# QuantumSavory/LDPCDecoders.jl

Hardware: AMD Instinct MI355X
Metric: decoded syndromes/sec (batchdecode!, 50 iters) + achieved HBM GB/s fraction (higher is better)
Workload: dtype f64

## Files before the change

### include/ldpc_mi355x_debug.h

```cpp
#ifndef LDPC_MI355X_DEBUG_H
#define LDPC_MI355X_DEBUG_H

#include "ldpc_mi355x.h"

#ifdef __cplusplus
extern "C" {
#endif

ldpc_status ldpc_debug_team_plan(int64_t nnz, int64_t max_iters, int64_t batch, int32_t cache_mib, int32_t rows_dv,
                                 int32_t out[6]);

ldpc_status ldpc_debug_team_rows(int64_t s, int64_t n, const int64_t *colptr, const int64_t *rowval, int32_t members,
                                 int32_t regs_per_wave, int32_t static_quarters, int32_t *degrees, int32_t *shape,
                                 int32_t *vtab, int32_t *ctab, int32_t *lds_edge, int32_t *reg_edge);

ldpc_status ldpc_debug_team_irr(int64_t s, int64_t n, const int64_t *colptr, const int64_t *rowval, int32_t members,
                                int32_t dc_bucket, int32_t dv_bucket, int32_t *shape, int32_t *ctab2, int32_t *ptab, int32_t *ploc,
                                int32_t *lds_edge, int32_t *posmap);

ldpc_status ldpc_debug_tile_plan(int64_t s, int64_t n, int64_t rec_words, int32_t relay, int32_t kernel_variant, int32_t *tier,
                                 int32_t *tile_syndromes, int64_t *state_bytes);

ldpc_status ldpc_debug_priors_tile_plan(int64_t s, int64_t n, int64_t rec_words, int32_t schedule, int32_t kernel_variant,
                                        int32_t *tier, int32_t *tile_syndromes, int64_t *state_bytes);

ldpc_status ldpc_debug_pauli_tile_plan(int64_t s, int64_t n, int64_t rec_words, int32_t kernel_variant, int32_t *tier,
                                       int32_t *tile_syndromes, int64_t *state_bytes);

#include "ldpc_mi355x_decim_debug.h"

#include "ldpc_mi355x_pauli_relay_debug.h"

ldpc_status ldpc_debug_layer_plan(int64_t s, int64_t n, const int64_t *colptr, const int64_t *rowval, int32_t *layer_of,
                                  int32_t *K);

ldpc_status ldpc_debug_bpots_plan(int64_t s, int64_t n, int64_t nnz, int32_t max_cdeg, int32_t max_bdeg, int32_t force_node,
                                  int32_t *kernel, int32_t *logS, int64_t *lds_bytes, int32_t *budget_kib, int32_t *dc, int32_t *dv);

ldpc_status ldpc_debug_bpots_last_launch(const ldpc_bpots_decoder *dec, int32_t *path, int64_t *groups, int32_t *grid,
                                         int32_t *chunk, int32_t *per_cu);

void *ldpc_debug_process_state(void);
ldpc_status ldpc_debug_adopt_process_state(void *state);

ldpc_status ldpc_debug_div_check(int64_t count, const double *num, const double *den, double *out_core, double *out_ieee);

ldpc_status ldpc_debug_llr_check(int64_t count, const double *odds, double *out_fast, double *out_lib);

#ifdef __cplusplus
}
#endif
#endif
```

### ldpcdecoders.jl_amd/_capi.py

```python
from __future__ import annotations

import ctypes
import os
import subprocess

_HERE = os.path.dirname(os.path.abspath(__file__))
CSRC = os.path.join(_HERE, "csrc")
LIB_PATH = os.environ.get("LDPC_MI355X_LIB") or os.path.join(CSRC, "libldpc_mi355x.so")
EXP_LIB_PATH = os.environ.get("LDPC_MI355X_EXP_LIB") or os.path.join(CSRC, "libldpc_mi355x_exp.so")

LDPC_OK = 0
STATUS_NAMES = {
    0: "LDPC_OK",
    1: "LDPC_ERR_INVALID_ARGUMENT",
    2: "LDPC_ERR_NO_DEVICE",
    3: "LDPC_ERR_HIP",
    4: "LDPC_ERR_OUT_OF_MEMORY",
    5: "LDPC_ERR_UNSUPPORTED",
}

MULTI_MAX_DEVICES = 16
EXCHANGE_AUTO, EXCHANGE_COPY, EXCHANGE_RCCL, EXCHANGE_NONE = 0, 1, 2, 3


# ... 201 lines not shown
    "ldpc_debug_process_state": (vp, []),
    "ldpc_debug_adopt_process_state": (i32, [vp]),
    "ldpc_debug_team_irr": (i32, [i64, i64, vp, vp, i32, i32, i32, P(i32 * 2), vp, vp, vp, vp, vp]),
    "ldpc_debug_llr_check": (i32, [i64, vp, vp, vp]),
    "ldpc_debug_tile_plan": (i32, [i64, i64, i64, i32, i32, P(i32), P(i32), P(i64)]),
    "ldpc_debug_layer_plan": (i32, [i64, i64, vp, vp, vp, P(i32)]),
    "ldpc_debug_priors_tile_plan": (i32, [i64, i64, i64, i32, i32, P(i32), P(i32), P(i64)]),
    "ldpc_debug_pauli_tile_plan": (i32, [i64, i64, i64, i32, P(i32), P(i32), P(i64)]),
    "ldpc_debug_bpots_plan": (i32, [i64, i64, i64, i32, i32, i32, P(i32), P(i32), P(i64), P(i32), P(i32), P(i32)]),
    "ldpc_debug_bpots_last_launch": (i32, [vp, P(i32), P(i64), P(i32), P(i32), P(i32)]),
}
DECIM_API = {
    "ldpc_decim_create": (i32, [i64, i64, i64, vp, vp, vp, i64, i64, P(DecimOptions), P(vp)]),
    "ldpc_decim_destroy": (i32, [vp]),
    "ldpc_decim_kernel": (i32, [vp]),
    "ldpc_decim_tile_syndromes": (i32, [vp]),
    "ldpc_decim_last_grid": (i32, [vp]),
    "ldpc_decim_decode_batch": (i32, [vp, i64, vp, vp, vp, vp, vp, vp]),
    "ldpc_decim_decode_batch_device": (i32, [vp, i64, vp, vp, vp, vp, vp, vp, vp]),
}
DECIM_DEBUG_API = {
    "ldpc_debug_decim_tile_plan": (i32, [i64, i64, i64, i32, P(i32), P(i32), P(i64)]),
}
OSD_SEARCH_API = {
    "ldpc_osd_set_search": (i32, [vp, i32, i64, i64, vp]),
    "ldpc_osd_search_method": (i32, [vp]),
    "ldpc_osd_search_weight": (i64, [vp, i64]),
}
PAULI_RELAY_API = {
    "ldpc_pauli_relay_create": (i32, [i64, P(CSSPattern), P(CSSPattern), vp, vp, vp, i64, vp, vp, P(PauliRelayOptions), P(vp)]),
    "ldpc_pauli_relay_destroy": (i32, [vp]),
    "ldpc_pauli_relay_kernel": (i32, [vp]),
    "ldpc_pauli_relay_tile_syndromes": (i32, [vp]),
    "ldpc_pauli_relay_last_grid": (i32, [vp]),
    "ldpc_pauli_relay_decode_batch": (i32, [vp, i64, vp, vp, vp, vp, vp, vp, vp, vp]),
    "ldpc_pauli_relay_decode_batch_device": (i32, [vp, i64, vp, vp, vp, vp, vp, vp, vp, vp, vp]),
}
PAULI_RELAY_DEBUG_API = {
    "ldpc_debug_pauli_relay_tile_plan": (i32, [i64, i64, i64, i32, P(i32), P(i32), P(i64)]),
}
EXPORTED_SYMBOLS = tuple(API)
DEBUG_SYMBOLS = tuple(DEBUG_API)
DECIM_SYMBOLS = tuple(DECIM_API)
DECIM_DEBUG_SYMBOLS = tuple(DECIM_DEBUG_API)
OSD_SEARCH_SYMBOLS = tuple(OSD_SEARCH_API)
PAULI_RELAY_SYMBOLS = tuple(PAULI_RELAY_API)
PAULI_RELAY_DEBUG_SYMBOLS = tuple(PAULI_RELAY_DEBUG_API)


def build(force: bool = False) -> str:
    subprocess.check_call(["make", "-s", "-C", CSRC, "all"])
    return LIB_PATH


_LIBS = {}


def _one_hip_runtime() -> None:
    if os.environ.get("LDPC_MI355X_NO_TORCH_PRELOAD"):
        return
    try:
        import torch
    except Exception:
        pass


def lib(experiments: bool = False) -> ctypes.CDLL:
    if experiments in _LIBS:
        return _LIBS[experiments]
    path = EXP_LIB_PATH if experiments else LIB_PATH
    if not os.path.exists(path):
        raise LdpcError(2, f"{path} is not built; run `python -c 'import __graft_entry__ as g; g.build()'` "
                           "or `make -C ldpcdecoders.jl_amd/csrc`. There is no CPU fallback.")
    _one_hip_runtime()
    L = ctypes.CDLL(path)
    for group in (API, DEBUG_API, DECIM_API, DECIM_DEBUG_API, OSD_SEARCH_API, PAULI_RELAY_API, PAULI_RELAY_DEBUG_API):
        for name, (restype, argtypes) in group.items():
            fn = getattr(L, name)
            fn.restype, fn.argtypes = restype, argtypes
    other = _LIBS.get(not experiments)
    if other is not None and os.path.realpath(path) != os.path.realpath(EXP_LIB_PATH if not experiments else LIB_PATH):
        check(L.ldpc_debug_adopt_process_state(other.ldpc_debug_process_state()), L)
    _LIBS[experiments] = L
    return L


def knobs_in_env() -> bool:
    return any(k.startswith("LDPC_") and not k.startswith("LDPC_MI355X_") for k in os.environ)


def lib_for(experiments=None) -> ctypes.CDLL:
    return lib(knobs_in_env() if experiments is None else bool(experiments))


def check(status: int, L: ctypes.CDLL = None) -> None:
    if status != LDPC_OK:
        raise LdpcError(status, (L or lib()).ldpc_last_error().decode("utf-8", "replace"))
```

### ldpcdecoders.jl_amd/csrc/bp_team_kernels.hpp

```cpp
#pragma once
#include "bp_kernels.hpp"

#ifndef LDPC_TEAM_ROWS_WIDE
#define LDPC_TEAM_ROWS_WIDE 1
#endif
#ifndef LDPC_TEAM_TFORM
#define LDPC_TEAM_TFORM 1
#endif
#ifndef LDPC_TEAM_TEST_DIRECT
#define LDPC_TEAM_TEST_DIRECT 1
#endif
#ifndef LDPC_TEAM_SLEEP
#define LDPC_TEAM_SLEEP 16
#endif

namespace ldpc {


template <int DV>
struct TeamVRec {
    int pos[DV], lrow[DV], bit;
};
template <int DV>
__device__ __forceinline__ TeamVRec<DV> team_vrec_load(const int *__restrict__ vt)
// ... 67 lines not shown

struct TeamParams {
    TeamRows rows;
    int G;
    int xcds;
    int nteams;
    int pre;
    int pairs;
    int dynamic;
    unsigned int *ctl;
    u64 *mism;
    int mism_stride;
    unsigned int *fault;
    int always_release;
    int scatter;
    unsigned int count_max;
    int inject_fault;
    unsigned int ticket;
    unsigned int rollcall_ticks;
    u64 *errmask_alt;
    int ahead_min;
    int ahead_from;
    int llr_raw;
};
constexpr unsigned int kTeamRollcallFailed = 0x80000000u;

constexpr int kTeamCtlMember = 64;
constexpr int kTeamCtlWords = 64 + 32 * kTeamMaxMembers;

#ifndef LDPC_TEAM_BARRIER_COUNTER
#define LDPC_TEAM_BARRIER_COUNTER 0
#endif
__device__ __forceinline__ bool team_barrier(unsigned int *ctl, int G, int rank, unsigned int k, unsigned int *fault,
                                             unsigned int ticket, int *sh_ok, bool one_xcd, unsigned int *sh_deal)
{
    asm volatile("s_waitcnt vmcnt(0)" ::: "memory");
    __syncthreads();
    if (threadIdx.x == 0) {
        if (!one_xcd) {
            __builtin_amdgcn_fence(__ATOMIC_RELEASE, "agent");
            asm volatile("s_waitcnt vmcnt(0)" ::: "memory");
        }
        int ok = 1;
        const unsigned int prev = __hip_atomic_fetch_add(ctl, 1u, __ATOMIC_RELAXED, __HIP_MEMORY_SCOPE_AGENT);
        const bool on_counter = LDPC_TEAM_BARRIER_COUNTER && one_xcd;
        if (prev + 1u == k * (unsigned)G) {
            if (!on_counter)
                for (int m = 0; m < G; ++m)
// ... 461 lines not shown
    if (team >= nteams || team >= ntiles) return;
    const int gw = rank * W + w, GW = G * W;
    unsigned int *const ctr = tp.ctl + (size_t)team * kTeamCtlWords;
    unsigned int *const xccs = ctr + 32;
    unsigned int *const tile_queue = tp.ctl + (size_t)nteams * kTeamCtlWords;
    unsigned int epoch = 0;
    __shared__ int sh_one_xcd;
#if LDPC_TEAM_FAULT_BLOCKS
    if (tp.inject_fault == 2 && team == 0 && rank == G - 1) return;
#endif
    if (!team_rollcall(ctr + 36, G, tp.fault, tp.ticket, tp.rollcall_ticks, &sh_ok)) return;
    if (threadIdx.x == 0) {
        unsigned int xcc;
        asm volatile("s_getreg_b32 %0, hwreg(HW_REG_XCC_ID)" : "=s"(xcc));
        __hip_atomic_fetch_or(xccs, 1u << (xcc & 15u), __ATOMIC_RELAXED, __HIP_MEMORY_SCOPE_AGENT);
    }
    bool one_xcd = false, placed = false;
    constexpr bool resumed = RESUMED;
    const BPCold *const cd = p.cold;
    u64 tk_check = 0, tk_var = 0, tk_rest = 0;
    int horizon = p.max_iters;
    long long tot_iters = 0;

    for (int tile = team; tile < ntiles;) {
    double *const Mt = p.msg + (size_t)(resumed ? tile : team) * (size_t)p.slot_stride + lane;
    u64 *const mw = tp.mism + (size_t)tile * (size_t)tp.mism_stride;
    const u64 *syn = synmask + (size_t)tile * s;
    u64 *em = p.errmask + (size_t)tile * n;
    u64 *fin = p.finmask + (size_t)tile * n;
    const long long b0 = (long long)tile * kTile;
    const long long left = batch - b0;
    u64 deferred = 0;
    const u64 valid = left >= kTile ? ~0ull : ((1ull << left) - 1ull);
    const u64 never = nevermask[tile];
    u64 active = valid;
    const int it0 = (resumed && ((valid >> lane) & 1ull)) ? cd->it0[b0 + lane] : 0;
    int my_iters = 0, my_conv = 0, it = 0;

    const bool can_run_ahead = !resumed && tp.errmask_alt != nullptr && tp.ahead_min > 0;
    u64 *const em_even = em, *const em_odd = can_run_ahead ? tp.errmask_alt + (size_t)tile * n : em;
    bool have_check = false;
    bool quiet = true;

    auto check_sweep = [&](const bool first, const int skip = 0) {
        const int nch = (s + kTeamCheckChunk - 1) / kTeamCheckChunk;
        auto chunk = [&](int c) {
            const int i1 = min(s, (c + 1) * kTeamCheckChunk);
            if constexpr (LROWS) {
                typedef int v4i __attribute__((ext_vector_type(4)));
                typedef int v8i __attribute__((ext_vector_type(8)));
                constexpr int FULL = (1 << DC) - 1;
                auto one = [&](double *const M, const v4i ct, const double sg) {
                    if (RR > 0 && ct.z == FULL) {
                        if (first) check_update_regs<DC, true, TF>(ct.w, sg, r, rget, rput);
                        else check_update_regs<DC, false, TF>(ct.w, sg, r, rget, rput);
                    } else if (ct.x == FULL) {
                        if (first) check_update_exact<DC, true, TF>(Lr + (size_t)ct.y * kTile, sg, r);
                        else check_update_exact<DC, false, TF>(Lr + (size_t)ct.y * kTile, sg, r);
                    } else if (RR > 0 && ct.z != 0) {
                        if (first) check_update_onchip<DC, true, TF>(M, Lr + (size_t)ct.y * kTile, Ldummy, (unsigned int)ct.x, (unsigned int)ct.z, ct.w, sg, r, rget, rput);
                        else check_update_onchip<DC, false, TF>(M, Lr + (size_t)ct.y * kTile, Ldummy, (unsigned int)ct.x, (unsigned int)ct.z, ct.w, sg, r, rget, rput);
                    } else if (first) {
                        check_update_mixed<DC, true, TF>(M, Lr + (size_t)ct.y * kTile, (unsigned int)ct.x, sg, r);
                    } else if (ct.x == 0) {
                        check_update_exact<DC, false, TF>(M, sg, r);
                    } else {
                        check_update_mixed<DC, false, TF>(M, Lr + (size_t)ct.y * kTile, (unsigned int)ct.x, sg, r);
                    }
                };
                const int i = c * kTeamCheckChunk;
                if (LDPC_HOT(kTeamCheckChunk == 2 && i + 2 == i1)) {
                    const v8i ct = *(const v8i *)(col_ptr + 4 * i);
                    const u64 s0 = syn[i], s1 = syn[i + 1];
                    const double sg0 = ((s0 >> lane) & 1ull) ? -1.0 : 1.0, sg1 = ((s1 >> lane) & 1ull) ? -1.0 : 1.0;
                    double *const M0 = Mt + (size_t)i * DC * kTile, *const M1 = M0 + (size_t)DC * kTile;
                    if ((ct.s0 | ct.s2 | ct.s4 | ct.s6) == 0 && !first && tp.pairs) {
                        check_update_pair<DC, TF>(M0, M1, sg0, sg1);
                    } else {
                        one(M0, v4i{ct.s0, ct.s1, ct.s2, ct.s3}, sg0);
                        one(M1, v4i{ct.s4, ct.s5, ct.s6, ct.s7}, sg1);
                    }
                    return;
                }
                for (int ii = i; ii < i1; ++ii) {
                    const v4i ct = *(const v4i *)(col_ptr + 4 * ii);
                    one(Mt + (size_t)ii * DC * kTile, ct, ((syn[ii] >> lane) & 1ull) ? -1.0 : 1.0);
                }
                return;
            }
            if constexpr (IRR) {
                for (int i = c * kTeamCheckChunk; i < i1; ++i) {
                    const int e0 = row_ptr[2 * i], lb = row_ptr[2 * i + 1];
                    const int deg = row_ptr[2 * i + 2] - e0;
                    const double sigma = ((syn[i] >> lane) & 1ull) ? -1.0 : 1.0;
                    double *const M = lb >= 0 ? Lr + (size_t)lb * kTile : Mt + (size_t)e0 * kTile;
                    if (first) check_update<DC, true, true>(M, deg, sigma, r);
                    else check_update<DC, false, true>(M, deg, sigma, r);
// ... 2 lines not shown
            }
            if (kTeamCheckChunk == 2 && !first && tp.pairs && i1 == c * 2 + 2) {
                const int i = c * 2;
                const int e0 = row_ptr[i], e1 = row_ptr[i + 1], e2 = row_ptr[i + 2];
                if (e1 - e0 == DC && e2 - e1 == DC) {
                    const double sg0 = ((syn[i] >> lane) & 1ull) ? -1.0 : 1.0, sg1 = ((syn[i + 1] >> lane) & 1ull) ? -1.0 : 1.0;
                    check_update_pair<DC>(Mt + (size_t)e0 * kTile, Mt + (size_t)e1 * kTile, sg0, sg1);
                    return;
                }
            }
            for (int i = c * kTeamCheckChunk; i < i1; ++i) {
                const int e0 = row_ptr[i];
                const int deg = row_ptr[i + 1] - e0;
                const double sigma = ((syn[i] >> lane) & 1ull) ? -1.0 : 1.0;
                if (first) check_update<DC, true>(Mt + (size_t)e0 * kTile, deg, sigma, r);
                else check_update<DC, false>(Mt + (size_t)e0 * kTile, deg, sigma, r);
            }
        };
        const int mine = (nch - rank + G - 1) / G;
        const int stat = LROWS ? tp.rows.static_c : W;
        const int mirror = (LROWS && (tp.rows.flip & 1) && w >= W / 2) ? 2 * w + stat - W : -1;
        for (int l = w; l < mine;) {
            const int lc = (mirror >= 0 && l < stat) ? mirror - l : l;
            if (!(LROWS && lc < skip * W)) chunk(lc * G + rank);
            l = !tp.dynamic ? l + W : (l + W < stat ? l + W : stat + team_deal(&sh_deal[0], lane));
        }
    };
    auto check_pre = [&](const int pre) {
        if constexpr (LROWS) {
            typedef int v4i __attribute__((ext_vector_type(4)));
            constexpr int FULL = (1 << DC) - 1;
            for (int k = 0; k < pre; ++k) {
                const int c = (w + k * W) * G + rank;
                for (int i = c * kTeamCheckChunk; i < (c + 1) * kTeamCheckChunk; ++i) {
                    const v4i ct = *(const v4i *)(col_ptr + 4 * i);
                    const double sg = ((syn[i] >> lane) & 1ull) ? -1.0 : 1.0;
                    if (RR > 0 && ct.z == FULL) check_update_regs<DC, false, TF>(ct.w, sg, r, rget, rput);
                    else check_update_exact<DC, false, TF>(Lr + (size_t)ct.y * kTile, sg, r);
                }
            }
        }
    };
    auto var_sweep = [&](const bool first = false) {
        const int vb = (one_xcd || LROWS || IRR) ? 4 : 16;
        const int nch = (n + vb - 1) / vb;
        const bool cap_on = WANT_LLR && (tp.llr_raw == 4 || tp.llr_raw == 5) && ((active >> lane) & 1ull);
        const size_t cap_rows = ((size_t)n + 3) & ~(size_t)3;
        unsigned int *const cap32 = (unsigned int *)p.llr + (size_t)tile * cap_rows * kTile;
        double *const cap64 = p.llr + (size_t)tile * cap_rows * kTile;
        auto cap_at = [&](int pos) { return ((size_t)(pos >> 2) * kTile + lane) * 4 + (size_t)(pos & 3); };
        auto capture1 = [&](int pos, double T) {
            if (!cap_on) return;
            if (tp.llr_raw == 4) cap32[cap_at(pos)] = llr_hi32(T);
            else cap64[cap_at(pos)] = T;
        };
        auto capture2 = [&](int pos, double T0, double T1) {
            if (!cap_on) return;
            typedef unsigned int v2u __attribute__((ext_vector_type(2)));
            typedef double v2d __attribute__((ext_vector_type(2)));
            if (tp.llr_raw == 4) *(v2u *)(cap32 + cap_at(pos)) = v2u{llr_hi32(T0), llr_hi32(T1)};
            else *(v2d *)(cap64 + cap_at(pos)) = v2d{T0, T1};
        };
        auto capture4 = [&](int pos, const double (&T)[4]) {
            if (!cap_on) return;
            typedef unsigned int v4u __attribute__((ext_vector_type(4)));
            typedef double v2d __attribute__((ext_vector_type(2)));
            if (tp.llr_raw == 4) *(v4u *)(cap32 + cap_at(pos)) = v4u{llr_hi32(T[0]), llr_hi32(T[1]), llr_hi32(T[2]), llr_hi32(T[3])};
            else { *(v2d *)(cap64 + cap_at(pos)) = v2d{T[0], T[1]}; *(v2d *)(cap64 + cap_at(pos) + 2) = v2d{T[2], T[3]}; }
        };
        auto decide = [&](int pos, int j, double T, bool cap = true) {
            const u64 dec = __ballot(T >= 1.0);
            if (WANT_LLR) {
                if (tp.llr_raw >= 4) { if (cap) capture1(pos, T); }
                else if (tp.llr_raw == 0 && ((active >> lane) & 1ull)) p.llr[((size_t)tile * n + j) * kTile + lane] = llr_of(T, p.llr_exact);
            }
            if (lane == 0) em[j] = dec;
        };
        auto chunk = [&](int c) {
            const int j1 = min(n, (c + 1) * vb);
            int j = c * vb;
            if constexpr (LROWS) {
                constexpr int VT = team_vtab_words(DV);
                if constexpr (kFuseFirst) {
                    if (first) {
                        if (j + 4 == j1) {
                            const int *const vt = csc2csr + (size_t)j * VT;
                            const TeamVRec<DV> A = team_vrec_load<DV>(vt), B = team_vrec_load<DV>(vt + VT), C = team_vrec_load<DV>(vt + 2 * VT),
                                               D = team_vrec_load<DV>(vt + 3 * VT);
                            double T[4];
                            T[0] = bit_update_first<DV, DC, TF>(Mt, Lr, sh_first, syn, lane, A.pos, A.lrow, r, rput);
                            T[1] = bit_update_first<DV, DC, TF>(Mt, Lr, sh_first, syn, lane, B.pos, B.lrow, r, rput);
                            T[2] = bit_update_first<DV, DC, TF>(Mt, Lr, sh_first, syn, lane, C.pos, C.lrow, r, rput);
                            T[3] = bit_update_first<DV, DC, TF>(Mt, Lr, sh_first, syn, lane, D.pos, D.lrow, r, rput);
                            decide(j, A.bit & 0x7fffffff, T[0], false);
                            decide(j + 1, B.bit & 0x7fffffff, T[1], false);
                            decide(j + 2, C.bit & 0x7fffffff, T[2], false);
                            decide(j + 3, D.bit & 0x7fffffff, T[3], false);
                            capture4(j, T);
                            return;
                        }
                        for (; j < j1; ++j) {
                            const TeamVRec<DV> A = team_vrec_load<DV>(csc2csr + (size_t)j * VT);
                            decide(j, A.bit & 0x7fffffff, bit_update_first<DV, DC, TF>(Mt, Lr, sh_first, syn, lane, A.pos, A.lrow, r, rput));
                        }
                        return;
                    }
                }
                auto single = [&](const TeamVRec<DV> &a, const int pa) {
                    if (a.bit >= 0) { decide(pa, a.bit, bit_update_exact_v<DV, TF>(Mt, a.pos, r)); return; }
                    if constexpr (RR > 0) {
                        int lo = a.lrow[0];
// ... 7 lines not shown
                    int rest = -1;
#pragma unroll
                    for (int k = 1; k < DV; ++k) rest &= a.lrow[k] & b.lrow[k];
                    if ((a.bit | b.bit) >= 0 && tp.pairs) {
                        double T0, T1;
                        bit_update_pair_v<DV, TF>(Mt, a.pos, b.pos, r, T0, T1);
                        decide(pa, a.bit, T0, false);
                        decide(pa + 1, b.bit, T1, false);
                        capture2(pa, T0, T1);
                    } else if (rest == -1 && tp.pairs) {
                        double T0, T1;
                        bit_update_pair_first<DV, TF>(Mt, Lr, a.pos, a.lrow[0], b.pos, b.lrow[0], r, rget, rput, T0, T1);
                        decide(pa, a.bit & 0x7fffffff, T0, false);
                        decide(pa + 1, b.bit & 0x7fffffff, T1, false);
                        capture2(pa, T0, T1);
                    } else {
                        single(a, pa);
                        single(b, pa + 1);
                    }
                };
                int q = j;
                if (LDPC_HOT(q + 4 == j1)) {
                    const int *const vt = csc2csr + (size_t)q * VT;
                    const TeamVRec<DV> A = team_vrec_load<DV>(vt), B = team_vrec_load<DV>(vt + VT), C = team_vrec_load<DV>(vt + 2 * VT),
                                       D = team_vrec_load<DV>(vt + 3 * VT);
                    if (LDPC_HOT(tp.pairs & 2)) {
                        int rest = -1;
#pragma unroll
                        for (int k = 1; k < DV; ++k) rest &= A.lrow[k] & B.lrow[k] & C.lrow[k] & D.lrow[k];
                        if (LDPC_HOT(rest == -1)) {
                            int ps[4][DV];
#pragma unroll
                            for (int k = 0; k < DV; ++k) { ps[0][k] = A.pos[k]; ps[1][k] = B.pos[k]; ps[2][k] = C.pos[k]; ps[3][k] = D.pos[k]; }
                            const int lc[4] = {A.lrow[0], B.lrow[0], C.lrow[0], D.lrow[0]};
                            double T[4];
                            constexpr bool KINDS = LDPC_TEAM_CHUNK_KINDS < 0 ? DV == 3 : LDPC_TEAM_CHUNK_KINDS != 0;
                            const int lmin = min(min(lc[0], lc[1]), min(lc[2], lc[3])), lmax = max(max(lc[0], lc[1]), max(lc[2], lc[3]));
                            if (KINDS && RR > 0 && lmax <= -2) bit_update_multi_first<DV, 4, TF, 2>(Mt, Lr, ps, lc, r, rget, rput, T);
                            else if (KINDS && lmin >= 0) bit_update_multi_first<DV, 4, TF, 1>(Mt, Lr, ps, lc, r, rget, rput, T);
                            else bit_update_multi_first<DV, 4, TF, 0>(Mt, Lr, ps, lc, r, rget, rput, T);
                            decide(q, A.bit & 0x7fffffff, T[0], false);
                            decide(q + 1, B.bit & 0x7fffffff, T[1], false);
                            decide(q + 2, C.bit & 0x7fffffff, T[2], false);
                            decide(q + 3, D.bit & 0x7fffffff, T[3], false);
                            capture4(q, T);
                            return;
                        }
                    }
// ... 17 lines not shown
                    decide(j, bw & 0x7fffffff, T);
                }
                return;
            }
            for (; tp.pairs && j + 1 < j1; j += 2) {
                const int c0 = col_ptr[j], c1 = col_ptr[j + 1], c2 = col_ptr[j + 2];
                if (c1 - c0 != DV || c2 - c1 != DV) break;
                double T0, T1;
                bit_update_pair<DV>(Mt, csc2csr + c0, csc2csr + c1, r, T0, T1);
                decide(j, j, T0, false);
                decide(j + 1, j + 1, T1, false);
                capture2(j, T0, T1);
            }
            for (; j < j1; ++j) {
                const int c0 = col_ptr[j];
                const int deg = col_ptr[j + 1] - c0;
                decide(j, j, bit_update<DV>(Mt, csc2csr + c0, deg, r));
            }
        };
        const int mine = (nch - rank + G - 1) / G;
        const int stat = LROWS ? tp.rows.static_v : W;
        const int mirror = (LROWS && (tp.rows.flip & 2) && w >= W / 2) ? 2 * w + stat - W : -1;
        for (int l = w; l < mine;) {
            chunk(((mirror >= 0 && l < stat) ? mirror - l : l) * G + rank);
            l = !tp.dynamic ? l + W : (l + W < stat ? l + W : stat + team_deal(&sh_deal[1], lane));
        }
    };
    auto run_test = [&](const int it_t, const u64 *em_t) {
        u64 mism = 0;
#if LDPC_TEAM_TEST_SPREAD
        const int gt = w * G + rank;
#else
        const int gt = gw;
#endif
        for (int i = gt * 64 + lane; i < s; i += GW * 64) {
            u64 par = 0;
            const int e1 = LROWS ? (i + 1) * DC : row_ptr[RS * (i + 1)];
            for (int e = LROWS ? i * DC : row_ptr[RS * i]; e < e1; e += 8) {
                int jb[8];
#pragma unroll
                for (int q = 0; q < 8; ++q) jb[q] = (e + q < e1) ? edge_bit[e + q] : -1;
                u64 wv[8];
#pragma unroll
                for (int q = 0; q < 8; ++q) wv[q] = (jb[q] >= 0) ? em_t[jb[q]] : 0ull;
#pragma unroll
                for (int q = 0; q < 8; ++q) par ^= wv[q];
            }
            mism |= par ^ syn[i];
        }
        mism = wave_or(mism);
#if LDPC_TEAM_TEST_DIRECT
        if (lane == 0 && mism) __hip_atomic_fetch_or(&mw[it_t - 1], mism, __ATOMIC_RELAXED, __HIP_MEMORY_SCOPE_AGENT);
#else
        if (lane == 0) sh_mism[w] = mism;
        __syncthreads();
        if (threadIdx.x == 0) {
            u64 part = 0;
#pragma unroll
// ... 140 lines not shown
```

### ldpcdecoders.jl_amd/csrc/ldpc_mi355x.hip

```cpp
#include "../../include/ldpc_mi355x.h"
#include "../../include/ldpc_mi355x_debug.h"
#define LDPC_AUX_KERNELS 1
#include "bp_kernels.hpp"
#include "bp_lds_kernels.hpp"
#include "bp_node_kernels.hpp"
#include "bp_team_kernels.hpp"
#include "bit_io_kernels.hpp"
#include "pickers.hpp"
#include "team_plan.hpp"
#include "host_env.hpp"
#include "host_common.hpp"

#include <algorithm>
#include <atomic>
#include <cstdio>
#include <cstdlib>
#include <cstring>
#include <memory>
#include <mutex>
#include <new>
#include <string>
#include <thread>
#include <utility>
#include <vector>
// ... 225 lines not shown
    for (int wgs = want_llr ? 2 : 3; wgs >= 1; --wgs) {
        int best = -1;
        for (int l = 0; l <= 6; ++l)
            if ((lds_bytes_needed((int)s, (int)n, (int)nnz, 1 << l, want_llr) + 512) * (size_t)wgs <= kLds) best = l;
        if (best >= 0) return best;
    }
    return -1;
}

}

struct ldpc_bp_decoder {
    int64_t s = 0, n = 0, nnz = 0, max_iters = 0;
    double per = 0.0;
    int device = 0;
    int num_cus = 0;
    int max_cdeg = 0, max_bdeg = 0;
    int wpt_fixed = 0;
    int resident_fixed = 0;
    int last_threads = 512, last_grid = 0;
    int last_kernel = 0, last_team = 1;
    int last_lds_rows = 0;
    int last_rows_on_chip = 0;
    int rows_on_chip = 0;
    size_t ws_budget = 0;
    int blocks_cache[2][17];
    int variant = 0;
    bool node_ok = false;
    bool node_msg_lds = false;
    int node_split_check = 0, node_split_edge = 0;
    int64_t node_max_batch = 0;
    int64_t node_take_max = 0;
    DevBuf node_msg;
    DevBuf team_ws, team_ws_lvl[2];
    std::vector<int> h_csc2csr;
    std::vector<int> h_row_ptr, h_edge_bit, h_col_ptr, h_irr_c2r;
    int irr_G = 0, irr_R = 0, irr_on_chip = 0;
    int irr_dcb = 0;
    DevBuf irr_ctab, irr_ptab, irr_ploc, irr_lds_edge, irr_posmap;
    bool team_rows_on = true;
    int rows_dc = 0, rows_dv = 0;
    int rows_G = 0, rows_R = 0;
    int rows_first_c = 0;
    int rows_regs = 0, rows_static_c = 0, rows_static_v = 0;
    DevBuf rows_ctab, rows_vtab, rows_lds_edge, rows_reg_edge, rows_posmap;
    int team_regs = kTeamRegRows;
    bool team_pre_set = false;
    int team_pre = 2;
    int team_flip = 3;
    int team_static_quarters = 3;
    unsigned int *team_fault = nullptr, *team_fault_dev = nullptr;
    int team_per_cu_want = 2;
    int64_t team_min_rows = 2048;
    bool team_min_rows_set = false;
    bool team_no_margin = false, team_always_release = false, team_coop = false;
    int team_max = 32;
    bool team_max_set = false;
    size_t team_cache = (size_t)240 << 20;
    int team_xcds = 0;
    int team_dynamic = 1;
    int team_pairs = 3;
    int team_ahead_from = 1;
    bool team_ahead_set = false;
    bool llr_exact = false;
    int team_llr_raw = 4;
    bool team_llr_footprint = true;
    int team_ahead = 32;
    DevBuf done_ctr;
    void *lat_pin = nullptr;
    void *lat_pin_dev = nullptr;
    size_t lat_pin_cap = 0;
    unsigned lat_ticket = 0;
// ... 295 lines not shown
    d->resident_fixed = options ? std::max(options->resident_tiles, 0) : 0;
    d->defer_thresh = options ? options->defer_threshold : 0;
    if (d->defer_thresh > 48 || d->defer_thresh < -1) { delete d; return fail(LDPC_ERR_INVALID_ARGUMENT, "defer_threshold must be -1, 0 or 1..48"); }
    for (auto &row : d->blocks_cache)
        for (int &v : row) v = -1;
    d->llr_exact = options && options->llr_exact != 0;
    d->variant = options ? options->kernel_variant : 0;
    if (d->variant < 0 || d->variant > 4) { delete d; return fail(LDPC_ERR_INVALID_ARGUMENT, "kernel_variant must be 0 ... 4"); }
    if (const char *e = exp_env("LDPC_TEAM_INJECT_FAULT")) d->inject_fault = std::max(1, std::atoi(e));
    if (const char *e = exp_env("LDPC_TEAM_ROLLCALL_US")) d->rollcall_ticks = (unsigned)std::max(1, std::atoi(e)) * 100u;
    if (const char *e = exp_env("LDPC_TEAM_CACHE_MIB")) d->team_cache = (size_t)std::max(0, std::atoi(e)) << 20;
    if (const char *e = exp_env("LDPC_TEAM_CACHE_KIB")) d->team_cache = (size_t)std::max(0, std::atoi(e)) << 10;
    if (const char *e = exp_env("LDPC_TEAM_DYNAMIC")) d->team_dynamic = std::atoi(e) != 0;
    if (const char *e = exp_env("LDPC_TEAM_XCDS")) d->team_xcds = std::max(1, std::min(8, std::atoi(e)));
    if (const char *e = exp_env("LDPC_TEAM_PAIRS")) d->team_pairs = std::atoi(e) & 3;
    if (const char *e = exp_env("LDPC_TEAM_AHEAD")) { d->team_ahead = std::max(0, std::min(65, std::atoi(e))); d->team_ahead_set = true; }
    if (const char *e = exp_env("LDPC_TEAM_AHEAD_FROM")) d->team_ahead_from = std::max(1, std::atoi(e));
    if (const char *e = exp_env("LDPC_TEAM_LLR_RAW")) { const int v = std::atoi(e); if (v == 0 || v == 4 || v == 5 || v == 6) d->team_llr_raw = v; }
    if (d->llr_exact && d->team_llr_raw == 4) d->team_llr_raw = 5;
    if (const char *e = exp_env("LDPC_TEAM_LLR_FOOTPRINT")) d->team_llr_footprint = std::atoi(e) != 0;
    if (const char *e = exp_env("LDPC_TEAM_REGS")) d->team_regs = std::max(0, std::min(kTeamRegRows, std::atoi(e)));
    if (const char *e = exp_env("LDPC_TEAM_FLIP")) d->team_flip = std::atoi(e) & 3;
    if (const char *e = exp_env("LDPC_TEAM_PRE")) { d->team_pre = std::max(0, std::min(8, std::atoi(e))); d->team_pre_set = true; }
    if (const char *e = exp_env("LDPC_TEAM_STATIC")) d->team_static_quarters = std::max(0, std::min(4, std::atoi(e)));
    if (const char *e = exp_env("LDPC_TEAM_PER_CU")) d->team_per_cu_want = std::max(1, std::min(3, std::atoi(e)));
    if (const char *e = exp_env("LDPC_TEAM_MIN_ROWS")) { d->team_min_rows = std::max<int64_t>(1, std::atoll(e)); d->team_min_rows_set = true; }
    d->team_no_margin = exp_env("LDPC_TEAM_NO_MARGIN") != nullptr;
    d->team_always_release = exp_env("LDPC_TEAM_ALWAYS_RELEASE") != nullptr;
    d->team_coop = exp_env("LDPC_TEAM_COOP_LAUNCH") != nullptr;
    if (const char *e = exp_env("LDPC_TEAM_MAX")) { d->team_max = std::max(1, std::min(kTeamMaxMembers, std::atoi(e))); d->team_max_set = true; }
    {
        void *fp = nullptr, *fd = nullptr;
        if (hipHostMalloc(&fp, 64, hipHostMallocMapped | hipHostMallocCoherent) != hipSuccess ||
            hipHostGetDevicePointer(&fd, fp, 0) != hipSuccess) {
            (void)hipGetLastError();
            if (fp) (void)hipHostFree(fp);
            delete d;
            return fail(LDPC_ERR_OUT_OF_MEMORY, "hipHostMalloc of the fault word failed");
        }
        std::memset(fp, 0, 64);
        d->team_fault = (unsigned int *)fp;
        d->team_fault_dev = (unsigned int *)fd;
    }
    d->lds_logS[0] = lds_logS(s, n, nnz, false);
    d->lds_logS[1] = lds_logS(s, n, nnz, true);
    if (const char *e = exp_env("LDPC_LDS_LOGS")) {
// ... 68 lines not shown
    return st;
}

ldpc_status ldpc_bp_get_info(const ldpc_bp_decoder *d, ldpc_bp_info *info)
{
    if (!d || !info) return fail(LDPC_ERR_INVALID_ARGUMENT, "NULL argument");
    std::memset(info, 0, sizeof *info);
    info->s = d->s; info->n = d->n; info->nnz = d->nnz; info->max_iters = d->max_iters; info->per = d->per;
    info->max_check_degree = d->max_cdeg; info->max_bit_degree = d->max_bdeg;
    info->device = d->device; info->tile_syndromes = kTile; info->waves_per_tile = d->last_threads / 64;
    info->resident_tiles = d->last_grid;
    const DevBuf *all[] = {&d->row_ptr, &d->edge_bit, &d->col_ptr, &d->csc2csr, &d->msg, &d->ctrl, &d->synmask,
                           &d->nevermask, &d->errmask, &d->finmask, &d->llr_t, &d->st_all, &d->node_msg, &d->pipe_dev[0], &d->pipe_dev[1], &d->pipe_dev[2],
                           &d->lvl_state[0], &d->lvl_state[1], &d->lvl_list[0], &d->lvl_list[1], &d->lvl_it[0], &d->lvl_it[1],
                           &d->lvl_syn[0], &d->lvl_syn[1], &d->lvl_never[0], &d->lvl_never[1], &d->lvl_err[0], &d->lvl_err[1], &d->lvl_fin[0], &d->lvl_fin[1],
                           &d->lvl_llr[0], &d->lvl_llr[1], &d->team_ws, &d->team_ws_lvl[0], &d->team_ws_lvl[1],
                           &d->rows_ctab, &d->rows_vtab, &d->rows_lds_edge, &d->rows_reg_edge, &d->rows_posmap,
                           &d->irr_ctab, &d->irr_ptab, &d->irr_ploc, &d->irr_lds_edge, &d->irr_posmap, &d->bits_syn, &d->bits_err};
    for (const DevBuf *b : all) info->workspace_bytes += (int64_t)b->cap;
    info->last_kernel = d->last_kernel;
    info->last_team_size = d->last_team;
    info->last_lds_rows = d->last_lds_rows;
    info->last_rows_on_chip = d->last_rows_on_chip;
    return LDPC_OK;
}

}

namespace {
struct ProcessState {
    std::mutex team_mu;
    hipEvent_t team_ev[64] = {};
};
ProcessState g_own_state;
ProcessState *g_ps = &g_own_state;
}
extern "C" void *ldpc_debug_process_state(void) { return g_ps; }
extern "C" ldpc_status ldpc_debug_adopt_process_state(void *state)
{
    if (!state) return fail(LDPC_ERR_INVALID_ARGUMENT, "state is NULL");
    g_ps = (ProcessState *)state;
    return LDPC_OK;
}

static size_t team_lds_bytes()
{
// ... 477 lines not shown
            bp_kernel_t kq = pick_kernel(d->max_cdeg, d->max_bdeg, want_llr, wpt * 64);
            int nb = 0;
            if (hipOccupancyMaxActiveBlocksPerMultiprocessor(&nb, (const void *)kq, wpt * 64, 0) != hipSuccess || nb <= 0) {
                (void)hipGetLastError();
                nb = 1;
            }
            bc = nb;
        }
        int slots = d->resident_fixed ? d->resident_fixed : bc * d->num_cus;
        slots = std::max(1, std::min(slots, max_slots));
        threads = wpt * 64;
        grid = std::min(slots, ntiles);
    }
    const TeamPlan plan = team_plan(d, batch, want_llr);
    const int team = plan.G;
    const int tile_grid = grid, tile_threads = threads;
    if (team > 1) { threads = 512; grid = plan.nteams; }
    d->last_threads = threads;
    const bool team_scatter = team > 1 && (exp_env("LDPC_TEAM_SCATTER") || plan.scatter);
    const int team_grid = team > 1 ? (team_scatter ? plan.nteams * team : plan.grid) : 0;
    d->last_grid = team > 1 ? plan.nteams * team : grid;
    d->last_kernel = team > 1 ? 4 : 1;
    d->last_team = team;
    d->last_lds_rows = 0; d->last_rows_on_chip = 0;
    const size_t slot_stride_bytes = std::max<size_t>((size_t)d->nnz, 1) * kTile * sizeof(double) + slot_pad_bytes();
    if ((st = ensure_workspace(d, (size_t)grid * slot_stride_bytes, grid, slot_stride_bytes, stream)) != LDPC_OK)
        return st;

    const int T0 = (d->defer_thresh < 0 || d->max_iters < 4 || ntiles < 2) ? 0
                   : (d->defer_thresh ? d->defer_thresh : d->defer_t0);
    struct Level {
        int thresh_in = 0;
        int cap_tiles = 0;
        unsigned int *count = nullptr;
        unsigned int *tile_queue = nullptr, *node_queue = nullptr;
        unsigned node_take = 0;
        unsigned team_cap = 0;
        int t_per_xcd = 0, t_gcap = 0, t_G = 0, t_nteams = 0, t_grid = 0, t_xcds = 8;
    } lv[3];
    int nlevels = 0;
    if (T0 > 0) {
        lv[1].thresh_in = T0;
        const int worst1 = (int)(((int64_t)ntiles * T0 + kTile - 1) / kTile) + 1;
        lv[1].cap_tiles = d->lvl_cap_force > 0 ? d->lvl_cap_force : std::min(worst1, std::max(8, std::max(grid, tile_grid) / 3));
        nlevels = 1;
        const int T1 = d->defer_t1;
        if (T1 > 0 && (lv[1].cap_tiles >= 8 || d->lvl_cap_force > 0)) {
// ... 153 lines not shown
                tp.rows.lds_edge = (const int *)d->irr_lds_edge.p;
                tp.rows.R = d->irr_R;
                tp.rows.reg_edge = nullptr; tp.rows.regs = 0;
                tp.rows.static_c = tp.rows.static_v = LDPC_TEAM_THREADS / 64; tp.rows.flip = 0;
                t_row = (const int *)d->irr_ctab.p;
                t_col = (const int *)d->irr_ptab.p;
                t_c2r = (const int *)d->irr_ploc.p;
                llr_posmap = (const int *)d->irr_posmap.p;
            }
        }
        if (plan.rows && team_rows_build(d, team) == LDPC_OK) {
            team_kernel_t tkr = pick_team_kernel_rows(d->rows_dc, d->rows_dv, want_llr, d->rows_regs > 0);
            const size_t need = (size_t)(d->rows_R + (d->rows_regs > 0 ? 1 : 0)) * kTile * sizeof(double);
            int occ_rows = 0;
            if (tkr && d->prepare_kernel((const void *)tkr, LDPC_TEAM_THREADS, need, &occ_rows) == LDPC_OK && occ_rows >= 1) {
                tk = tkr; team_lds = need;
                d->last_lds_rows = d->rows_R; d->last_rows_on_chip = d->rows_on_chip;
                tp.rows.lds_edge = (const int *)d->rows_lds_edge.p;
                tp.rows.R = d->rows_R;
                tp.rows.reg_edge = (const int *)d->rows_reg_edge.p;
                tp.rows.regs = d->rows_regs;
                tp.rows.static_c = d->rows_static_c; tp.rows.static_v = d->rows_static_v; tp.rows.flip = d->team_flip;
                tp.rows.first_c = d->rows_first_c;
                tp.pre = std::min((plan.wide && !d->team_pre_set) ? 8 : d->team_pre, d->rows_first_c / (LDPC_TEAM_THREADS / 64));
                t_col = (const int *)d->rows_ctab.p;
                t_c2r = (const int *)d->rows_vtab.p;
                llr_posmap = (const int *)d->rows_posmap.p;
            }
        }
        const u64 *a_syn = (const u64 *)d->synmask.p, *a_nev = (const u64 *)d->nevermask.p;
        void *args[] = {&p, &tp, &t_row, &a_eb, &t_col, &t_c2r, &a_syn, &a_nev};
        const hipError_t te = launch_team_grid(d, tk, team_grid, args, stream, team_lds);
        if (te != hipSuccess) {
            (void)hipGetLastError();
            d->team_max = 1;
            threads = tile_threads; grid = tile_grid;
            d->last_kernel = 1; d->last_team = 1; d->last_lds_rows = 0; d->last_rows_on_chip = 0; d->last_grid = grid; d->last_threads = threads;
            if ((st = ensure_workspace(d, (size_t)grid * slot_stride_bytes, grid, slot_stride_bytes, stream)) != LDPC_OK) return st;
            p.msg = (double *)d->msg.p;
            kfn = pick_kernel(d->max_cdeg, d->max_bdeg, want_llr, threads);
            team_ran = false;
            llr_raw_out = 0;
            llr_posmap = nullptr;
        }
        if (team_ran && exp_env("LDPC_TEAM_DEBUG")) {
            const int nt = std::min(plan.nteams, ntiles);
            std::vector<unsigned> xm((size_t)nt);
            (void)ldpc_detail::wait_stream(stream, d->device, "LDPC_TEAM_DEBUG (stream synchronise)");
            for (int t = 0; t < nt; ++t)
                (void)hipMemcpy(&xm[(size_t)t], tp.ctl + (size_t)t * kTeamCtlWords + 32, sizeof(unsigned), hipMemcpyDeviceToHost);
            int single = 0;
            for (unsigned v : xm) single += __builtin_popcount(v) == 1;
            std::fprintf(stderr, "[ldpc] team kernel: %d tiles, %d teams x %d workgroups, grid %d; %d teams on one XCD (first masks %x %x %x)\n",
                         ntiles, plan.nteams, team, team_grid, single, xm[0], nt > 1 ? xm[1] : 0u, nt > 2 ? xm[2] : 0u);
            for (int t = 0; t < nt; ++t) {
                std::vector<unsigned> ml((size_t)team * 32);
                (void)hipMemcpy(ml.data(), tp.ctl + (size_t)t * kTeamCtlWords + kTeamCtlMember, ml.size() * sizeof(unsigned), hipMemcpyDeviceToHost);
                double sc = 0, sv = 0; unsigned cmin = ~0u, cmax = 0, vmin = ~0u, vmax = 0; int cm = 0, vm = 0;
                for (int m = 0; m < team; ++m) {
                    const unsigned c = ml[(size_t)m * 32 + 1], v = ml[(size_t)m * 32 + 2];
// ... 586 lines not shown
```

Baseline: 94020.

## Keep static team-kernel index tables and syndrome bits resident in registers

In the LROWS team kernel, each wave now loads once, before the tile loop, the check-node column tables, variable-node CSC-to-CSR records and parity-test edge indices for its statically assigned chunks. These are held in VGPRs spread across lanes, and the check sweep, bit sweep, pre-pass and convergence test read them back with readlane instead of reloading from global memory every iteration. Syndrome bits for the resident check chunks are also packed into a per-tile register mask. The aim is to cut repeated index-table traffic and latency, at the cost of more register pressure and possibly lower occupancy. A debug query and an env knob are added, and the feature is on by default.

```diff
diff --git a/include/ldpc_mi355x_debug.h b/include/ldpc_mi355x_debug.h
--- a/include/ldpc_mi355x_debug.h
+++ b/include/ldpc_mi355x_debug.h
@@ -40,6 +40,8 @@
 ldpc_status ldpc_debug_bpots_last_launch(const ldpc_bpots_decoder *dec, int32_t *path, int64_t *groups, int32_t *grid,
                                          int32_t *chunk, int32_t *per_cu);
 
+#include "ldpc_mi355x_team_debug.h"
+
 void *ldpc_debug_process_state(void);
 ldpc_status ldpc_debug_adopt_process_state(void *state);
 
diff --git a/include/ldpc_mi355x_team_debug.h b/include/ldpc_mi355x_team_debug.h
--- /dev/null
+++ b/include/ldpc_mi355x_team_debug.h
@@ -0,0 +1,10 @@
+#ifndef LDPC_MI355X_TEAM_DEBUG_H
+#define LDPC_MI355X_TEAM_DEBUG_H
+
+#ifndef LDPC_MI355X_DEBUG_H
+#error "include ldpc_mi355x_debug.h, which includes this file"
+#endif
+
+ldpc_status ldpc_debug_team_resident(const ldpc_bp_decoder *dec, int32_t out[6]);
+
+#endif
diff --git a/ldpcdecoders.jl_amd/_capi.py b/ldpcdecoders.jl_amd/_capi.py
--- a/ldpcdecoders.jl_amd/_capi.py
+++ b/ldpcdecoders.jl_amd/_capi.py
@@ -247,6 +247,9 @@
 DECIM_DEBUG_API = {
     "ldpc_debug_decim_tile_plan": (i32, [i64, i64, i64, i32, P(i32), P(i32), P(i64)]),
 }
+TEAM_DEBUG_API = {
+    "ldpc_debug_team_resident": (i32, [vp, P(i32 * 6)]),
+}
 OSD_SEARCH_API = {
     "ldpc_osd_set_search": (i32, [vp, i32, i64, i64, vp]),
     "ldpc_osd_search_method": (i32, [vp]),
@@ -268,6 +271,7 @@
 DEBUG_SYMBOLS = tuple(DEBUG_API)
 DECIM_SYMBOLS = tuple(DECIM_API)
 DECIM_DEBUG_SYMBOLS = tuple(DECIM_DEBUG_API)
+TEAM_DEBUG_SYMBOLS = tuple(TEAM_DEBUG_API)
 OSD_SEARCH_SYMBOLS = tuple(OSD_SEARCH_API)
 PAULI_RELAY_SYMBOLS = tuple(PAULI_RELAY_API)
 PAULI_RELAY_DEBUG_SYMBOLS = tuple(PAULI_RELAY_DEBUG_API)
@@ -299,7 +303,7 @@
                            "or `make -C ldpcdecoders.jl_amd/csrc`. There is no CPU fallback.")
     _one_hip_runtime()
     L = ctypes.CDLL(path)
-    for group in (API, DEBUG_API, DECIM_API, DECIM_DEBUG_API, OSD_SEARCH_API, PAULI_RELAY_API, PAULI_RELAY_DEBUG_API):
+    for group in (API, DEBUG_API, TEAM_DEBUG_API, DECIM_API, DECIM_DEBUG_API, OSD_SEARCH_API, PAULI_RELAY_API, PAULI_RELAY_DEBUG_API):
         for name, (restype, argtypes) in group.items():
             fn = getattr(L, name)
             fn.restype, fn.argtypes = restype, argtypes
diff --git a/ldpcdecoders.jl_amd/csrc/bp_team_kernels.hpp b/ldpcdecoders.jl_amd/csrc/bp_team_kernels.hpp
--- a/ldpcdecoders.jl_amd/csrc/bp_team_kernels.hpp
+++ b/ldpcdecoders.jl_amd/csrc/bp_team_kernels.hpp
@@ -113,8 +113,11 @@
     int ahead_min;
     int ahead_from;
     int llr_raw;
+    int resident;
 };
 constexpr unsigned int kTeamRollcallFailed = 0x80000000u;
+constexpr int kTeamCtlResident = 40;
+constexpr int kTeamResCheckChunks = 32, kTeamResPosChunks = 16;
 
 constexpr int kTeamCtlMember = 64;
 constexpr int kTeamCtlWords = 64 + 32 * kTeamMaxMembers;
@@ -622,6 +625,61 @@
     int horizon = p.max_iters;
     long long tot_iters = 0;
 
+    constexpr bool kRes = LROWS && !(WANT_LLR && RR > 0);
+    constexpr int kResV = kRes ? 2 * DV + 1 : 1, kResT = kRes ? DC : 1;
+    int res_v[kResV] = {}, res_c[4] = {}, res_t[kResT] = {};
+    int nres_v = 0, nres_c = 0;
+    bool res_test = false;
+#if LDPC_TEAM_TEST_SPREAD
+    const int gt = w * G + rank;
+#else
+    const int gt = gw;
+#endif
+    if constexpr (kRes) {
+        if (tp.resident & 1) {
+            constexpr int VT = team_vtab_words(DV);
+            const int mine_v = ((n + 3) / 4 - rank + G - 1) / G, stat_v = min(tp.rows.static_v, mine_v);
+            const int mine_c = ((s + kTeamCheckChunk - 1) / kTeamCheckChunk - rank + G - 1) / G, stat_c = min(tp.rows.static_c, mine_c);
+            nres_v = min(kTeamResPosChunks, max(0, (stat_v - w + W - 1) / W));
+            nres_c = min(kTeamResCheckChunks, max(0, (stat_c - w + W - 1) / W));
+            const int jv = (((w + (lane >> 2) * W) * G + rank) << 2) + (lane & 3);
+            const bool on_v = (lane >> 2) < nres_v && jv < n;
+#pragma unroll
+            for (int k = 0; k < kResV; ++k) res_v[k] = on_v ? csc2csr[(size_t)jv * VT + k] : 0;
+            const int ic = ((w + (lane >> 1) * W) * G + rank) * kTeamCheckChunk + (lane & 1);
+            const bool on_c = (lane >> 1) < nres_c && ic < s;
+#pragma unroll
+            for (int k = 0; k < 4; ++k) res_c[k] = on_c ? col_ptr[4 * (size_t)ic + k] : 0;
+        }
+        if ((tp.resident & 2) && s <= GW * 64) {
+            res_test = true;
+            const int i = gt * 64 + lane;
+#pragma unroll
+            for (int q = 0; q < DC; ++q) res_t[q] = i < s ? edge_bit[(size_t)i * DC + q] : 0;
+        }
+#pragma unroll
+        for (int k = 0; k < kResV; ++k) asm volatile("" : "+v"(res_v[k]));
+#pragma unroll
+        for (int k = 0; k < 4; ++k) asm volatile("" : "+v"(res_c[k]));
+#pragma unroll
+        for (int q = 0; q < kResT; ++q) asm volatile("" : "+v"(res_t[q]));
+        if (team == 0 && rank == 0 && threadIdx.x == 0) {
+            ctr[kTeamCtlResident] = (unsigned)nres_c; ctr[kTeamCtlResident + 1] = (unsigned)nres_v; ctr[kTeamCtlResident + 2] = res_test ? 1u : 0u;
+        }
+    }
+    auto res_vrec = [&](const int at) {
+        TeamVRec<DV> rc;
+        if constexpr (kRes) {
+#pragma unroll
+            for (int k = 0; k < DV; ++k) {
+                rc.pos[k] = __builtin_amdgcn_readlane(res_v[k], at);
+                rc.lrow[k] = __builtin_amdgcn_readlane(res_v[DV + k], at);
+            }
+            rc.bit = __builtin_amdgcn_readlane(res_v[2 * DV], at);
+        }
+        return rc;
+    };
+
     for (int tile = team; tile < ntiles;) {
     double *const Mt = p.msg + (size_t)(resumed ? tile : team) * (size_t)p.slot_stride + lane;
     u64 *const mw = tp.mism + (size_t)tile * (size_t)tp.mism_stride;
@@ -636,6 +694,14 @@
     u64 active = valid;
     const int it0 = (resumed && ((valid >> lane) & 1ull)) ? cd->it0[b0 + lane] : 0;
     int my_iters = 0, my_conv = 0, it = 0;
+    u64 res_syn = 0;
+    if constexpr (kRes) {
+        for (int k = 0; k < nres_c; ++k) {
+            const int i = ((w + k * W) * G + rank) * kTeamCheckChunk;
+            if (i < s) res_syn |= ((syn[i] >> lane) & 1ull) << (2 * k);
+            if (i + 1 < s) res_syn |= ((syn[i + 1] >> lane) & 1ull) << (2 * k + 1);
+        }
+    }
 
     const bool can_run_ahead = !resumed && tp.errmask_alt != nullptr && tp.ahead_min > 0;
     u64 *const em_even = em, *const em_odd = can_run_ahead ? tp.errmask_alt + (size_t)tile * n : em;
@@ -644,7 +710,7 @@
 
     auto check_sweep = [&](const bool first, const int skip = 0) {
         const int nch = (s + kTeamCheckChunk - 1) / kTeamCheckChunk;
-        auto chunk = [&](int c) {
+        auto chunk = [&](int c, const int kres = -1) {
             const int i1 = min(s, (c + 1) * kTeamCheckChunk);
             if constexpr (LROWS) {
                 typedef int v4i __attribute__((ext_vector_type(4)));
@@ -670,9 +736,21 @@
                 };
                 const int i = c * kTeamCheckChunk;
                 if (LDPC_HOT(kTeamCheckChunk == 2 && i + 2 == i1)) {
-                    const v8i ct = *(const v8i *)(col_ptr + 4 * i);
-                    const u64 s0 = syn[i], s1 = syn[i + 1];
-                    const double sg0 = ((s0 >> lane) & 1ull) ? -1.0 : 1.0, sg1 = ((s1 >> lane) & 1ull) ? -1.0 : 1.0;
+                    v8i ct;
+                    double sg0, sg1;
+                    if (kres >= 0) {
+                        const int a0 = 2 * kres, a1 = a0 + 1;
+                        ct = v8i{__builtin_amdgcn_readlane(res_c[0], a0), __builtin_amdgcn_readlane(res_c[1], a0), __builtin_amdgcn_readlane(res_c[2], a0),
+                                 __builtin_amdgcn_readlane(res_c[3], a0), __builtin_amdgcn_readlane(res_c[0], a1), __builtin_amdgcn_readlane(res_c[1], a1),
+                                 __builtin_amdgcn_readlane(res_c[2], a1), __builtin_amdgcn_readlane(res_c[3], a1)};
+                        sg0 = ((res_syn >> a0) & 1ull) ? -1.0 : 1.0;
+                        sg1 = ((res_syn >> a1) & 1ull) ? -1.0 : 1.0;
+                    } else {
+                        ct = *(const v8i *)(col_ptr + 4 * i);
+                        const u64 s0 = syn[i], s1 = syn[i + 1];
+                        sg0 = ((s0 >> lane) & 1ull) ? -1.0 : 1.0;
+                        sg1 = ((s1 >> lane) & 1ull) ? -1.0 : 1.0;
+                    }
                     double *const M0 = Mt + (size_t)i * DC * kTile, *const M1 = M0 + (size_t)DC * kTile;
                     if ((ct.s0 | ct.s2 | ct.s4 | ct.s6) == 0 && !first && tp.pairs) {
                         check_update_pair<DC, TF>(M0, M1, sg0, sg1);
@@ -721,7 +799,8 @@
         const int mirror = (LROWS && (tp.rows.flip & 1) && w >= W / 2) ? 2 * w + stat - W : -1;
         for (int l = w; l < mine;) {
             const int lc = (mirror >= 0 && l < stat) ? mirror - l : l;
-            if (!(LROWS && lc < skip * W)) chunk(lc * G + rank);
+            const int kres = (kRes && l < stat && ((lc - w) / W) < nres_c) ? (lc - w) / W : -1;
+            if (!(LROWS && lc < skip * W)) chunk(lc * G + rank, kres);
             l = !tp.dynamic ? l + W : (l + W < stat ? l + W : stat + team_deal(&sh_deal[0], lane));
         }
     };
@@ -732,8 +811,17 @@
             for (int k = 0; k < pre; ++k) {
                 const int c = (w + k * W) * G + rank;
                 for (int i = c * kTeamCheckChunk; i < (c + 1) * kTeamCheckChunk; ++i) {
-                    const v4i ct = *(const v4i *)(col_ptr + 4 * i);
-                    const double sg = ((syn[i] >> lane) & 1ull) ? -1.0 : 1.0;
+                    v4i ct;
+                    double sg;
+                    if (kRes && k < nres_c) {
+                        const int at = kTeamCheckChunk * k + (i - c * kTeamCheckChunk);
+                        ct = v4i{__builtin_amdgcn_readlane(res_c[0], at), __builtin_amdgcn_readlane(res_c[1], at), __builtin_amdgcn_readlane(res_c[2], at),
+                                 __builtin_amdgcn_readlane(res_c[3], at)};
+                        sg = ((res_syn >> at) & 1ull) ? -1.0 : 1.0;
+                    } else {
+                        ct = *(const v4i *)(col_ptr + 4 * i);
+                        sg = ((syn[i] >> lane) & 1ull) ? -1.0 : 1.0;
+                    }
                     if (RR > 0 && ct.z == FULL) check_update_regs<DC, false, TF>(ct.w, sg, r, rget, rput);
                     else check_update_exact<DC, false, TF>(Lr + (size_t)ct.y * kTile, sg, r);
                 }
@@ -775,7 +863,7 @@
             }
             if (lane == 0) em[j] = dec;
         };
-        auto chunk = [&](int c) {
+        auto chunk = [&](int c, const int kres = -1) {
             const int j1 = min(n, (c + 1) * vb);
             int j = c * vb;
             if constexpr (LROWS) {
@@ -784,8 +872,12 @@
                     if (first) {
                         if (j + 4 == j1) {
                             const int *const vt = csc2csr + (size_t)j * VT;
-                            const TeamVRec<DV> A = team_vrec_load<DV>(vt), B = team_vrec_load<DV>(vt + VT), C = team_vrec_load<DV>(vt + 2 * VT),
-                                               D = team_vrec_load<DV>(vt + 3 * VT);
+                            TeamVRec<DV> A, B, C, D;
+                            if (kres >= 0) {
+                                A = res_vrec(4 * kres); B = res_vrec(4 * kres + 1); C = res_vrec(4 * kres + 2); D = res_vrec(4 * kres + 3);
+                            } else {
+                                A = team_vrec_load<DV>(vt); B = team_vrec_load<DV>(vt + VT); C = team_vrec_load<DV>(vt + 2 * VT); D = team_vrec_load<DV>(vt + 3 * VT);
+                            }
                             double T[4];
                             T[0] = bit_update_first<DV, DC, TF>(Mt, Lr, sh_first, syn, lane, A.pos, A.lrow, r, rput);
                             T[1] = bit_update_first<DV, DC, TF>(Mt, Lr, sh_first, syn, lane, B.pos, B.lrow, r, rput);
@@ -839,8 +931,12 @@
                 int q = j;
                 if (LDPC_HOT(q + 4 == j1)) {
                     const int *const vt = csc2csr + (size_t)q * VT;
-                    const TeamVRec<DV> A = team_vrec_load<DV>(vt), B = team_vrec_load<DV>(vt + VT), C = team_vrec_load<DV>(vt + 2 * VT),
-                                       D = team_vrec_load<DV>(vt + 3 * VT);
+                    TeamVRec<DV> A, B, C, D;
+                    if (kres >= 0) {
+                        A = res_vrec(4 * kres); B = res_vrec(4 * kres + 1); C = res_vrec(4 * kres + 2); D = res_vrec(4 * kres + 3);
+                    } else {
+                        A = team_vrec_load<DV>(vt); B = team_vrec_load<DV>(vt + VT); C = team_vrec_load<DV>(vt + 2 * VT); D = team_vrec_load<DV>(vt + 3 * VT);
+                    }
                     if (LDPC_HOT(tp.pairs & 2)) {
                         int rest = -1;
 #pragma unroll
@@ -904,18 +1000,25 @@
         const int stat = LROWS ? tp.rows.static_v : W;
         const int mirror = (LROWS && (tp.rows.flip & 2) && w >= W / 2) ? 2 * w + stat - W : -1;
         for (int l = w; l < mine;) {
-            chunk(((mirror >= 0 && l < stat) ? mirror - l : l) * G + rank);
+            const int lc = (mirror >= 0 && l < stat) ? mirror - l : l;
+            chunk(lc * G + rank, (kRes && l < stat && ((lc - w) / W) < nres_v) ? (lc - w) / W : -1);
             l = !tp.dynamic ? l + W : (l + W < stat ? l + W : stat + team_deal(&sh_deal[1], lane));
         }
     };
     auto run_test = [&](const int it_t, const u64 *em_t) {
         u64 mism = 0;
-#if LDPC_TEAM_TEST_SPREAD
-        const int gt = w * G + rank;
-#else
-        const int gt = gw;
-#endif
-        for (int i = gt * 64 + lane; i < s; i += GW * 64) {
+        if (kRes && res_test) {
+            const int i = gt * 64 + lane;
+            if (i < s) {
+                u64 wv[kResT], par = 0;
+#pragma unroll
+                for (int q = 0; q < kResT; ++q) wv[q] = em_t[res_t[q]];
+#pragma unroll
+                for (int q = 0; q < kResT; ++q) par ^= wv[q];
+                mism = par ^ syn[i];
+            }
+        }
+        for (int i = (kRes && res_test) ? s : gt * 64 + lane; i < s; i += GW * 64) {
             u64 par = 0;
             const int e1 = LROWS ? (i + 1) * DC : row_ptr[RS * (i + 1)];
             for (int e = LROWS ? i * DC : row_ptr[RS * i]; e < e1; e += 8) {
diff --git a/ldpcdecoders.jl_amd/csrc/ldpc_mi355x.hip b/ldpcdecoders.jl_amd/csrc/ldpc_mi355x.hip
--- a/ldpcdecoders.jl_amd/csrc/ldpc_mi355x.hip
+++ b/ldpcdecoders.jl_amd/csrc/ldpc_mi355x.hip
@@ -271,6 +271,7 @@
     int last_kernel = 0, last_team = 1;
     int last_lds_rows = 0;
     int last_rows_on_chip = 0;
+    int last_resident[3] = {-1, 0, 0};
     int rows_on_chip = 0;
     size_t ws_budget = 0;
     int blocks_cache[2][17];
@@ -297,6 +298,7 @@
     bool team_pre_set = false;
     int team_pre = 2;
     int team_flip = 3;
+    int team_resident = 3;
     int team_static_quarters = 3;
     unsigned int *team_fault = nullptr, *team_fault_dev = nullptr;
     int team_per_cu_want = 2;
@@ -638,6 +640,7 @@
     if (const char *e = exp_env("LDPC_TEAM_REGS")) d->team_regs = std::max(0, std::min(kTeamRegRows, std::atoi(e)));
     if (const char *e = exp_env("LDPC_TEAM_FLIP")) d->team_flip = std::atoi(e) & 3;
     if (const char *e = exp_env("LDPC_TEAM_PRE")) { d->team_pre = std::max(0, std::min(8, std::atoi(e))); d->team_pre_set = true; }
+    if (const char *e = exp_env("LDPC_TEAM_RESIDENT")) d->team_resident = std::atoi(e) & 3;
     if (const char *e = exp_env("LDPC_TEAM_STATIC")) d->team_static_quarters = std::max(0, std::min(4, std::atoi(e)));
     if (const char *e = exp_env("LDPC_TEAM_PER_CU")) d->team_per_cu_want = std::max(1, std::min(3, std::atoi(e)));
     if (const char *e = exp_env("LDPC_TEAM_MIN_ROWS")) { d->team_min_rows = std::max<int64_t>(1, std::atoll(e)); d->team_min_rows_set = true; }
@@ -752,6 +755,22 @@
     info->last_team_size = d->last_team;
     info->last_lds_rows = d->last_lds_rows;
     info->last_rows_on_chip = d->last_rows_on_chip;
+    return LDPC_OK;
+}
+
+ldpc_status ldpc_debug_team_resident(const ldpc_bp_decoder *d, int32_t out[6])
+{
+    if (!d || !out) return fail(LDPC_ERR_INVALID_ARGUMENT, "NULL argument");
+    for (int k = 0; k < 6; ++k) out[k] = 0;
+    if (d->last_resident[0] < 0 || !d->team_ws.p) return LDPC_OK;
+    DeviceGuard guard;
+    (void)hipSetDevice(d->device);
+    const ldpc_status st = ldpc_detail::wait_device(d->device, "ldpc_debug_team_resident (device synchronise)");
+    if (st != LDPC_OK) return st;
+    unsigned int held[3] = {0u, 0u, 0u};
+    LDPC_HIP_TRY(hipMemcpy(held, (const unsigned int *)d->team_ws.p + kTeamCtlResident, sizeof held, hipMemcpyDeviceToHost));
+    out[0] = d->last_resident[0]; out[1] = d->last_resident[1]; out[2] = d->last_resident[2];
+    out[3] = (int32_t)held[0]; out[4] = (int32_t)held[1]; out[5] = (int32_t)held[2];
     return LDPC_OK;
 }
 
@@ -1275,7 +1294,7 @@
     d->last_grid = team > 1 ? plan.nteams * team : grid;
     d->last_kernel = team > 1 ? 4 : 1;
     d->last_team = team;
-    d->last_lds_rows = 0; d->last_rows_on_chip = 0;
+    d->last_lds_rows = 0; d->last_rows_on_chip = 0; d->last_resident[0] = -1;
     const size_t slot_stride_bytes = std::max<size_t>((size_t)d->nnz, 1) * kTile * sizeof(double) + slot_pad_bytes();
     if ((st = ensure_workspace(d, (size_t)grid * slot_stride_bytes, grid, slot_stride_bytes, stream)) != LDPC_OK)
         return st;
@@ -1475,6 +1494,9 @@
                 tp.rows.regs = d->rows_regs;
                 tp.rows.static_c = d->rows_static_c; tp.rows.static_v = d->rows_static_v; tp.rows.flip = d->team_flip;
                 tp.rows.first_c = d->rows_first_c;
+                tp.resident = d->team_resident;
+                d->last_resident[0] = tp.resident;
+                d->last_resident[1] = d->rows_static_c / (LDPC_TEAM_THREADS / 64); d->last_resident[2] = d->rows_static_v / (LDPC_TEAM_THREADS / 64);
                 tp.pre = std::min((plan.wide && !d->team_pre_set) ? 8 : d->team_pre, d->rows_first_c / (LDPC_TEAM_THREADS / 64));
                 t_col = (const int *)d->rows_ctab.p;
                 t_c2r = (const int *)d->rows_vtab.p;
@@ -1488,7 +1510,7 @@
             (void)hipGetLastError();
             d->team_max = 1;
             threads = tile_threads; grid = tile_grid;
-            d->last_kernel = 1; d->last_team = 1; d->last_lds_rows = 0; d->last_rows_on_chip = 0; d->last_grid = grid; d->last_threads = threads;
+            d->last_kernel = 1; d->last_team = 1; d->last_lds_rows = 0; d->last_rows_on_chip = 0; d->last_resident[0] = -1; d->last_grid = grid; d->last_threads = threads;
             if ((st = ensure_workspace(d, (size_t)grid * slot_stride_bytes, grid, slot_stride_bytes, stream)) != LDPC_OK) return st;
             p.msg = (double *)d->msg.p;
             kfn = pick_kernel(d->max_cdeg, d->max_bdeg, want_llr, threads);
```

Result: no change. 93620 (-0.4%).
